# LeapLabTHU/LAUDNet

Hardware: AMD Instinct MI355X
Metric: images/sec, LAUD-ResNet101 @224 bs256 (dynamic-inference hot path) (higher is better)
Workload: dtype bf16x3 (fp32 tensors; each fp32 product = 3 bf16 MFMA products of hi/lo splits, fp32 accumulate)

## Files before the change

include/ldn_hip.h:

```cpp
#ifndef LDN_HIP_H
#define LDN_HIP_H

#include <stddef.h>
#include <stdint.h>

#ifdef __cplusplus
extern "C" {
#endif

#define LDN_OK 0
#define LDN_EINVAL (-1)
#define LDN_EHIP (-2)

const char* ldn_last_error(void);
int ldn_version(void);
int ldn_debug_violations(int* count, int* first_code, int reset);
int ldn_plan_timeouts(int* count, int reset);
const int* ldn_fault_flag(void);
int ldn_device_cus(int* cus);
#define LDN_MATH_DEFAULT (-1)
#define LDN_MATH_FP32 0
#define LDN_MATH_BF16X3 1
int ldn_default_math_mode(void);

// ... 91 lines not shown
                             const float* chan_mask, const int32_t* row_prefix, int B, const int32_t* m_count, int m_cap, int C, float* h,
                             int ldh, void* stream);

size_t ldn_rows_bn_postmask_bwd_workspace_bytes(int m_cap, int C, int B);
int ldn_rows_bn_postmask_bwd(const float* dz, int lddz, const float* u, int ldu, const float* h, int ldh, const float* mean, const float* invstd,
                             const float* gamma, const float* beta, const float* chan_mask, const int32_t* row_prefix, int B, const float* gate,
                             const float* dsq, const int32_t* m_count, int m_cap, int C, float* du, int lddu, float* d_gamma, float* d_beta,
                             float* g_mask, float* work, void* stream);

size_t ldn_rows_ln_bwd_workspace_bytes(int m_cap, int C);
int ldn_rows_ln_bwd(const float* x, int ldx, int rows, const float* stats, const float* gamma, const int32_t* list, const int32_t* count,
                    int m_cap, int C, const float* dy, int lddy, float* dx, int lddx, float* d_gamma, float* d_beta, float* xhat, int ldxh,
                    float* work, void* stream);

int ldn_conv_rows_pool(const float* a, int lda, const int32_t* a_rows, const int32_t* m_count, int m_cap, const void* w,
                       int cin, int cout, const float* scale, const float* shift, int relu, const int32_t* relu_if_neg,
                       const int32_t* out_rows, const float* residual, int ldr, float* out, int ldo, float* pool, int S,
                       int Sx, int Ho, int Wo, int math_mode, void* stream);

int ldn_conv_rows_ps(const float* a, int lda, int a_presplit, const int32_t* a_rows, const int32_t* m_count, int m_cap,
                     const void* w_split, int cin, int cout, const float* scale, const float* shift, int relu,
                     const int32_t* relu_if_neg, const int32_t* out_rows, const float* residual, int ldr, float* out, int ldo,
                     int out_presplit, float* pool, int S, int Sx, int Ho, int Wo, void* stream);
int ldn_conv3x3_rows_ps(const void* a_presplit, int lda, const int32_t* nbr, const int32_t* m_count, int m_cap, const void* w_split,
                        int cin, int cout, const float* scale, const float* shift, int relu, void* out, int ldo, int out_presplit,
                        int rows_hint, void* stream);
int ldn_row_stats(const float* x, int ld, int rows, int C, float eps, float* stats, void* stream);
int ldn_row_stats_list(const float* x, int ld, int rows, int C, float eps, const int32_t* list, const int32_t* count, float* stats,
                       void* stream);

int ldn_channel_masker_splits(int HW);
int ldn_channel_masker(const float* x, int B, int HW, int C, const float* w1, const float* b1, const float* w2,
                       const float* b2, int hidden, int G, int gran, const float* mask_in, float* mask,
                       float* logits, int32_t* ch_idx, int32_t* ch_cnt, float* work, const float* gap_partial,
                       int gap_splits, void* stream);
size_t ldn_channel_masker_workspace_bytes(int B, int HW, int C);

int ldn_forward_stats(const int32_t* cnt, int B, const float* denom, const float* st_in, int st_cols, const double* terms,
                      double static_flops, int n_blocks, float* st_out, float* perc, float* flops, void* stream);

int ldn_conv_image(const float* a, int lda, int B, int Hi, int Wi, int ksize, int stride, int Ho, int Wo,
                   const float* w, int cin, int cout, const int32_t* k_idx, const int32_t* k_cnt, int kgran,
                   const int32_t* n_idx, const int32_t* n_cnt, const float* scale, const float* shift,
                   int shift_classes, const float* post_sub, int relu, const float* residual, int ldr,
                   float* out, int ldo, float* colsum, int out_format, int math_mode, void* stream);

// ... 132 lines not shown
```

laudnet_amd/_lib.py:

```python
from __future__ import annotations

import ctypes as C
import os

import torch

_PKG = os.path.dirname(os.path.abspath(__file__))
LIB_PATH = os.environ.get("LDN_LIB_PATH", os.path.join(_PKG, "libldn_hip.so"))

_P = C.c_void_p
_I = C.c_int

SIGNATURES = {
    "ldn_last_error": ([], C.c_char_p),
    "ldn_version": ([], _I),
    "ldn_debug_violations": ([C.POINTER(_I), C.POINTER(_I), _I], _I),
    "ldn_plan_timeouts": ([C.POINTER(_I), _I], _I),
    "ldn_fault_flag": ([], C.POINTER(_I)),
    "ldn_device_cus": ([C.POINTER(_I)], _I),
    "ldn_default_math_mode": ([], _I),
    "ldn_spatial_masker": ([_P, _I, _I, _I, _I, _P, _P, _I, _I, _P, _P, _P, _P, _P, _P], _I),
    "ldn_spatial_masker_workspace_bytes": ([_I, _I, _I, _I, _I], C.c_size_t),
    "ldn_mask_to_index": ([_P, _I, _I, _I, _I, _I, _I, _P, _P, _P, _P, _P, _P, _P, _P, _P, _P, _P], _I),
    "ldn_mask_to_index_workspace_bytes": ([_I, _I, _I, _I], C.c_size_t),
    "ldn_mask_plan_fits": ([_I, _I, _I, _I, _I], _I),
    "ldn_hint_rows": ([_I], _I),
    "ldn_layer_index": ([_P, _I, _I, _I, _I, _I, _I, _P, _P, _P, _P, _P, _P, _P, _P, _P, _P], _I),
    "ldn_layer_head": ([_P, _I, _I, _I, _P, _P, _I, _P, _P, _P], _I),
    "ldn_mask_plan": ([_P, _P, _I, _P, _P, _P, _P, _I, _I, _I, _I, _I, _I, _I, _P, _P, _P, _P, _P, _P, _P, _P, _P, _P, _P], _I),
    "ldn_conv_rows_pool": ([_P, _I, _P, _P, _I, _P, _I, _I, _P, _P, _I, _P, _P, _P, _I, _P, _I, _P, _I, _I, _I, _I, _I, _P], _I),
    "ldn_conv_rows_ps": ([_P, _I, _I, _P, _P, _I, _P, _I, _I, _P, _P, _I, _P, _P, _P, _I, _P, _I, _I, _P, _I, _I, _I, _I, _P], _I),
    "ldn_conv3x3_rows_ps": ([_P, _I, _P, _P, _I, _P, _I, _I, _P, _P, _I, _P, _I, _I, _I, _P], _I),
    "ldn_gather_rows": ([_P, _I, _P, _P, _I, _I, _P, _I, _P], _I),
    "ldn_scatter_add_relu": ([_P, _I, _P, _P, _I, _I, _P, _I, _P, _I, _P], _I),
    "ldn_conv_rows": ([_P, _I, _P, _I, _P, _I, _P, _I, _I, _P, _P, _I, _P, _P, _P, _I, _P, _I, _I, _P], _I),
    "ldn_conv_rows_split": ([_P, _I, _P, _I, _P, _I, _P, _I, _I, _P, _P, _I, _P, _P, _P, _I, _P, _I, _P, _P, _I, _I, _P, _I, _I, _I,
                             _I, _I, _P, _P, _P], _I),
    "ldn_conv_rows_f32": ([_P, _I, _P, _I, _P, _I, _P, _I, _I, _P, _P, _I, _P, _P, _P, _I, _P, _I, _P, _P, _I, _I, _P, _I, _I, _I,
                             _I, _I, _P, _P, _P], _I),
    "ldn_wgrad_rows_ok": ([_I, _I, _I], _I),
    "ldn_wgrad_rows_workspace_bytes": ([_I, _I, _I, _I], C.c_size_t),
    "ldn_wgrad_rows": ([_P, _I, _P, _I, _I, _P, _I, _P, _I, _I, _I, _P, _P, _I, _P], _I),
    "ldn_wgrad_grouped_rows_ok": ([_I, _I], _I),
    "ldn_wgrad_grouped_rows_workspace_bytes": ([_I, _I, _I], C.c_size_t),
    "ldn_wgrad_grouped_rows": ([_P, _I, _P, _I, _I, _P, _P, _I, _I, _I, _P, _P, _I, _P], _I),
    "ldn_rows_chanmask": ([_P, _I, _P, _I, _P, _P, _I, _I, _P], _I),
    "ldn_rows_act_bwd_workspace_bytes": ([_I, _I, _I], C.c_size_t),
    "ldn_rows_act_bwd": ([_P, _I, _P, _I, _P, _P, _P, _P, _P, _I, _P, _I, _P, _I, _I, _P, _I, _P, _P, _P, _P, _P], _I),
    "ldn_rows_img_dot_workspace_bytes": ([_I, _I, _I], C.c_size_t),
    "ldn_rows_img_dot": ([_P, _I, _P, _I, _P, _I, _P, _I, _I, _P, _P, _P], _I),
    "ldn_rows_postmask_bwd_workspace_bytes": ([_I, _I, _I], C.c_size_t),
    "ldn_rows_postmask_bwd": ([_P, _I, _P, _I, _P, _P, _P, _P, _I, _P, _P, _P, _I, _I, _P, _I, _P, _P, _P, _P, _P], _I),
    "ldn_rows_bn_stats_workspace_bytes": ([_I, _I], C.c_size_t),
    "ldn_rows_bn_stats": ([_P, _I, _P, _P, _I, _P, _I, _I, C.c_float, _P, _P, _P, _P, _P], _I),
# ... 152 lines not shown
```

laudnet_amd/csrc/ldn_dense.hip:

```cpp
#include "ldn_common.h"
#include "ldn_dense_plan.h"
#include <type_traits>

namespace ldn {

struct DenseArgs {
    const float* a; int lda;
    const int32_t* a_rows; const int32_t* m_count; int m_cap;
    const unsigned char* ws;
    int cin, cout;
    const float* scale; const float* shift; int relu;
    const int32_t* relu_if_neg; const int32_t* out_rows;
    const float* residual; int ldr; float* out; int ldo;
    int taps;
    int shift_classes; const int32_t* pix_map;
    int Hi, Wi, Ho, Wo, stride;
    const float* post_sub;
    const float* chmask; int rows_per_img;
    int mtn, ntn;
    const float* ln_stats; const float* ln_c1;
    float* pool; int pool_gy, pool_gx, pool_Sx;
    const float* a_gate; int gate_rows;
};

__device__ __attribute__((aligned(16))) float g_dense_zero[2048] = {0.f};
#ifdef LDN_TRACE
__device__ unsigned long long* g_dense_trace = nullptr;
#define DT(x) x = __builtin_amdgcn_s_memtime();
#else
#define DT(x)
#endif

#ifndef LDN_DENSE_ABLATE
#define LDN_DENSE_ABLATE 0
#endif
__device__ __forceinline__ void dma16_abl(const void* gsrc, unsigned lds_base) {
#if LDN_DENSE_ABLATE & 1
    return;
#endif
#if LDN_DENSE_ABLATE & 2
    gsrc = g_dense_zero;
#endif
    dma16(gsrc, lds_base);
}

// ... 388 lines not shown
        DT(d5)
        a_wait += d1 - d0; a_bar += d2 - d1; a_issue += d3 - d2; a_prep += d4 - d3; a_mfma += d5 - d4;
#endif
    }
#undef LDN_DENSE_STEP
#ifdef LDN_TRACE
    DT(d_loop)
#endif
    wait_vm<0>();
    lds_barrier();
    if (!active) return;

    dense_epilogue<NSUB, T9, FULL, OF>(p, acc, s_arow, s_orow, s_cls, reinterpret_cast<float*>(s_ring + wave * 4096), wave, lane, n0, nsub);
#if defined(LDN_TRACE)
    if (g_dense_trace && lane == 0) {
        unsigned long long dend;
        DT(dend)
        unsigned long long* r = g_dense_trace + ((size_t)blockIdx.x * 8 + wave) * 8;
        r[0] = a_wait; r[1] = a_bar; r[2] = a_issue; r[3] = a_prep; r[4] = a_mfma; r[5] = d_loop - d_start; r[6] = dend - d_loop; r[7] = nchunks;
    }
#endif
}

template <int NSUB, bool T9, bool PS, bool OF, bool FEAT = false, bool RAG = false, bool AG = false>
__global__ __launch_bounds__(512, 2) void k_dense2(const DenseArgs p) {
    static_assert(!RAG || (!T9 && !PS && !OF), "the ragged form is the plain 1x1");
    static_assert(!AG || (!T9 && !PS), "the gated form reads fp32 rows of a 1x1");
    constexpr int NT = NSUB * 32;
    constexpr int KS = NSUB <= 4 ? 64 : 32;
    constexpr int SPS = KS / 32;
    constexpr int WROWB = KS * 4;
    constexpr int UPR = WROWB / 16;
    constexpr int RPI = 1024 / WROWB;
    constexpr int NWI = (NT + 8 * RPI - 1) / (8 * RPI);
    constexpr int WSLOT = NWI * 8 * 1024;
    constexpr int RSLOT = 32 * 128;
    constexpr int D_ROWS = 256, NST = 2 * NSUB;
    extern __shared__ __attribute__((aligned(16))) unsigned char smem[];
    int* const s_arow = reinterpret_cast<int*>(smem);
    int* const s_orow = s_arow + D_ROWS;
    int* const s_cls = s_orow + D_ROWS;
    int* const s_atap = s_cls + D_ROWS;
    unsigned char* const s_w = smem + (T9 ? 12 : 2) * D_ROWS * 4;
    unsigned char* const s_r = s_w + 2 * WSLOT;
    float* const s_gate = reinterpret_cast<float*>(s_r + 8 * 2 * RSLOT);

    const int tid = threadIdx.x, lane = tid & 63;
    const int wave = __builtin_amdgcn_readfirstlane(tid >> 6);
    const int l31 = lane & 31, h = lane >> 5;
    const int xcd = blockIdx.x & 7, slot_i = blockIdx.x >> 3;
    const int nt = slot_i % p.ntn, mt = (slot_i / p.ntn) * 8 + xcd;
    if (mt >= p.mtn) return;
    const int M = p.m_count ? min(p.m_count[0], p.m_cap) : p.m_cap;
    const int m0 = mt * D_ROWS;
    if (m0 >= M) return;
    const int rows = min(D_ROWS, M - m0);
    const int n0 = nt * NT;

    if (tid < D_ROWS) {
        int ar = -1, orw = -1;
        if (tid < rows) {
            ar = (p.a_rows && !T9) ? p.a_rows[m0 + tid] : m0 + tid;
            orw = p.out_rows ? p.out_rows[m0 + tid] : m0 + tid;
            if (p.relu == 1 || (p.relu == 2 && p.relu_if_neg[m0 + tid] < 0)) orw |= D_ROW_RELU;
        }
        int cls = 0;
        if (T9 && tid < rows && p.shift_classes > 1) {
            const int q = p.pix_map[m0 + tid] % (p.Ho * p.Wo);
            const int oy = q / p.Wo, ox = q - oy * p.Wo;
            const int top = oy * p.stride - 1 < 0, bot = oy * p.stride + 1 >= p.Hi;
            const int lef = ox * p.stride - 1 < 0, rig = ox * p.stride + 1 >= p.Wi;
            cls = ((top | (bot << 1)) * 4 + (lef | (rig << 1))) * p.cout;
        }
        LDN_DCHECK(tid >= rows || (ar >= -1 && (orw & (D_ROW_RELU - 1)) >= 0), 501);
        s_arow[tid] = ar;
        s_orow[tid] = orw;
        if (T9) s_cls[tid] = cls;
    }
    if (T9) {
        constexpr int NE = (D_ROWS * 9 + 511) / 512;
        int tv[NE];
#pragma unroll
        for (int u = 0; u < NE; ++u) {
            const int i = tid + 512 * u, r = i / 9;
            tv[u] = (i < D_ROWS * 9 && r < rows) ? p.a_rows[(size_t)(m0 + r) * 9 + (i - r * 9)] : -1;
        }
#pragma unroll
        for (int u = 0; u < NE; ++u)
            if (tid + 512 * u < D_ROWS * 9) s_atap[tid + 512 * u] = tv[u];
    }
    int goff = 0;
    if constexpr (AG) {
        const int gld = round_up(p.cin, 32), q4 = gld >> 2;
        const int slot0 = m0 / p.gate_rows, nsl = (m0 + rows - 1) / p.gate_rows - slot0 + 1;
        for (int i = tid; i < nsl * q4; i += 512) {
            const int sl = i / q4, k = (i - sl * q4) * 4;
            reinterpret_cast<f32x4*>(s_gate)[i] = k < p.cin ? *reinterpret_cast<const f32x4*>(p.a_gate + (size_t)(slot0 + sl) * p.cin + k) : f32x4{0.f, 0.f, 0.f, 0.f};
        }
        goff = ((m0 + min(wave * 32 + (lane & 31), rows - 1)) / p.gate_rows - slot0) * gld + 8 * (lane >> 5);
    }
// ... 7 lines not shown
    const unsigned lds_w = lds_off(s_w), lds_r = lds_off(s_r) + (unsigned)wave * 2u * RSLOT;
    unsigned char* const my_r = s_r + wave * 2 * RSLOT;
    const unsigned char* const zrow = reinterpret_cast<const unsigned char*>(g_dense_zero);

    const unsigned char* wsrc[NWI];
    int wku[NWI];
#pragma unroll
    for (int k = 0; k < NWI; ++k) {
        wku[k] = 0;
        const int rr = 8 * RPI * k + RPI * wave + lane / UPR;
        const int sw = UPR == 16 ? (rr & 15) : ((rr >> 1) & 7);
        wsrc[k] = (rr < NT && (!RAG || n0 + rr < p.cout)) ? p.ws + (long)(n0 + rr) * wrow + (((lane % UPR) ^ sw) << 4) : zrow;
        if (RAG) wku[k] = ((lane % UPR) ^ sw) * 4;
    }
    auto dma_w = [&](int S, int k) {
        const bool pad = NT % (8 * RPI) != 0 && 8 * RPI * k + RPI * wave >= NT;
        const int Sc = min(S, nstep - 1);
        const bool ktail = RAG && Sc * KS + wku[k] >= p.cin;
        dma16_abl(ktail ? zrow : wsrc[k] + (pad || wsrc[k] == zrow ? 0l : (long)Sc * WROWB),
                (unsigned)__builtin_amdgcn_readfirstlane((int)(lds_w + (unsigned)(S & 1) * WSLOT + (unsigned)(8 * RPI * k + RPI * wave) * WROWB)));
    };
    const unsigned char* rsrc[4];
    int tap_r = 0, ck_r = 0;
    auto load_tap = [&](int tap) {
#pragma unroll
        for (int k = 0; k < 4; ++k) {
            const int r = 8 * k + (lane >> 3);
            const int ar = T9 ? s_atap[(wave * 32 + r) * 9 + tap] : s_arow[wave * 32 + r];
            const unsigned char* base = ar >= 0 ? reinterpret_cast<const unsigned char*>(p.a) + (long)ar * p.lda * 4 : zrow;
            rsrc[k] = base + (((lane & 7) ^ ((r >> 1) & 7)) << 4);
        }
    };
    auto dma_r = [&](int s, int k) {
        const unsigned dst = (unsigned)__builtin_amdgcn_readfirstlane((int)(lds_r + (unsigned)(s & 1) * RSLOT + (unsigned)k * 1024u));
        if constexpr (RAG) {
            const int r = 8 * k + (lane >> 3);
            const int ku = ((lane & 7) ^ ((r >> 1) & 7)) * 4;
            dma16_abl(ck_r * 32 + ku < p.cin ? rsrc[k] + ck_r * 128 : zrow, dst);
        } else {
            dma16_abl(rsrc[k] + ck_r * 128, dst);
        }
    };
    auto next_r = [&]() {
        if constexpr (RAG) { ++ck_r; return; }
        if (++ck_r == cpt) {
            ck_r = 0;
            if (T9) {
                tap_r = min(tap_r + 1, 8);
                load_tap(tap_r);
            }
        }
    };

    if (!active) {
        for (int k = 0; k < NWI; ++k) dma_w(0, k);
        for (int S = 0; S < nstep; ++S) {
            wait_vm<0>();
            lds_barrier();
            for (int k = 0; k < NWI; ++k) dma_w(S + 1, k);
        }
        wait_vm<0>();
        return;
    }

    f32x16 acc[NSUB];
#pragma unroll
    for (int j = 0; j < NSUB; ++j)
#pragma unroll
        for (int r = 0; r < 16; ++r) acc[j][r] = 0.f;

    bf16x8 bh[2][2], bl[2][2];
    f32x4 raw[4];
// ... 160 lines not shown
LDN_DEFINE_TU_VIOLATIONS(tu_violations_dense)

static int launch_rows(void (*kernel)(const DenseArgs), const char* name, int r, int nt, unsigned threads, size_t lds, DenseArgs& a, hipStream_t st) {
    a.ntn = ceil_div(a.cout, nt);
    a.mtn = ceil_div(a.m_cap, r);
    LDN_REQUIRE(allow_dynamic_lds(reinterpret_cast<const void*>(kernel), lds), "%s: cannot reserve %zu B of LDS", name, lds);
    hipLaunchKernelGGL(kernel, dim3((unsigned)round_up(a.mtn, 8) * a.ntn), dim3(threads), lds, st, a);
    LDN_CHECK_LAUNCH(name);
    return LDN_OK;
}

template <int NSUB, bool T9, bool FULL, bool F32, int R, bool PS, bool OF>
static int launch_dense_f(DenseArgs& a, hipStream_t st) {
    constexpr int NT = NSUB * 32, D = (NSUB >= 6 || R == 128) ? 2 : 3;
    return launch_rows(&k_dense<NSUB, T9, FULL, F32, R, PS, OF>, "k_dense", R, NT, 2 * R, (size_t)(T9 ? 12 : 2) * R * 4 + (size_t)D * (R + NT) * 128, a, st);
}

template <int NSUB, bool T9, bool PS, bool OF, bool FEAT, bool RAG, bool AG>
static int launch_dense2(DenseArgs& a, hipStream_t st) {
    constexpr int NT = NSUB * 32, KS = NSUB <= 4 ? 64 : 32, WROWB = KS * 4, RPI = 1024 / WROWB, NWI = (NT + 8 * RPI - 1) / (8 * RPI);
    const size_t lds = (size_t)(T9 ? 12 : 2) * 256 * 4 + 2 * (size_t)NWI * 8 * 1024 + 8 * 2 * (size_t)32 * 128 +
                       (AG ? (size_t)dense_gate_bytes(a.gate_rows, a.cin) : 0);
    return launch_rows(&k_dense2<NSUB, T9, PS, OF, FEAT, RAG, AG>, "k_dense2", 256, NT, 512, lds, a, st);
}

static int launch_dense_plan(const DensePlan& plan, DenseArgs& a, hipStream_t st) {
#define LDN_D1(...) if (plan == LDN_DENSE_ROW1(__VA_ARGS__)) return launch_dense_f<__VA_ARGS__>(a, st);
#define LDN_D2(...) if (plan == LDN_DENSE_ROW2(__VA_ARGS__)) return launch_dense2<__VA_ARGS__>(a, st);
    LDN_DENSE_KERNELS(LDN_D1, LDN_D2)
#undef LDN_D1
#undef LDN_D2
    LDN_REQUIRE(false, "ldn_conv_rows: %s is not built (taps %d, cin %d, cout %d, m_cap %d)", dense_plan_name(plan).c_str(), a.taps, a.cin, a.cout, a.m_cap);
}

}

using namespace ldn;

#ifdef LDN_TRACE
extern "C" int ldn_debug_set_dense_trace(void* buf) {
    unsigned long long* q = static_cast<unsigned long long*>(buf);
    return hipMemcpyToSymbol(HIP_SYMBOL(g_dense_trace), &q, sizeof(q)) == hipSuccess ? 0 : -2;
}
#endif

static thread_local long g_rows_hint = -1;
// ... 37 lines not shown
    s.rows_known = dense_rows_known(d.m_cap, d.m_count != nullptr, hint);
    s.f32 = f.f32; s.ps = f.ps; s.of = f.of; s.pool = d.pool != nullptr;
    s.feat = d.post_sub || d.chmask || d.ln_stats || d.relu == 3;
    s.gated = d.a_gate != nullptr; s.gate_bytes = s.gated ? dense_gate_bytes(d.gate_rows, d.cin) : 0;
    return launch_dense_plan(dense_plan(s), d, static_cast<hipStream_t>(stream));
}

extern "C" int ldn_conv_rows_split(const float* a, int lda, const int32_t* a_rows, int taps, const int32_t* m_count, int m_cap,
                                   const void* w_split, int cin, int cout, const float* scale, const float* shift, int relu,
                                   const int32_t* relu_if_neg, const int32_t* out_rows, const float* residual, int ldr,
                                   float* out, int ldo, const float* post_sub, const float* chan_mask, int rows_per_image,
                                   int shift_classes, const int32_t* pix_map, int Hi, int Wi, int Ho, int Wo, int stride,
                                   const float* ln_stats, const float* ln_c1, void* stream) {
    DenseArgs d{};
    d.a = a; d.lda = lda; d.a_rows = a_rows; d.taps = taps; d.m_count = m_count; d.m_cap = m_cap;
    d.ws = static_cast<const unsigned char*>(w_split); d.cin = cin; d.cout = cout;
    d.scale = scale; d.shift = shift; d.relu = relu; d.relu_if_neg = relu_if_neg;
    d.out_rows = out_rows; d.residual = residual; d.ldr = ldr; d.out = out; d.ldo = ldo;
    d.post_sub = post_sub; d.chmask = chan_mask; d.rows_per_img = rows_per_image; d.ln_stats = ln_stats; d.ln_c1 = ln_c1;
    d.shift_classes = shift_classes; d.pix_map = pix_map; d.Hi = Hi; d.Wi = Wi; d.Ho = Ho; d.Wo = Wo; d.stride = stride;
    return conv_rows_dense(d, DenseForm{}, stream);
}

extern "C" int ldn_conv_rows_f32(const float* a, int lda, const int32_t* a_rows, int taps, const int32_t* m_count, int m_cap,
                                 const float* w, int cin, int cout, const float* scale, const float* shift, int relu,
                                 const int32_t* relu_if_neg, const int32_t* out_rows, const float* residual, int ldr,
                                 float* out, int ldo, const float* post_sub, const float* chan_mask, int rows_per_image,
                                 int shift_classes, const int32_t* pix_map, int Hi, int Wi, int Ho, int Wo, int stride,
                                 const float* ln_stats, const float* ln_c1, void* stream) {
    DenseArgs d{};
    d.a = a; d.lda = lda; d.a_rows = a_rows; d.taps = taps; d.m_count = m_count; d.m_cap = m_cap;
    d.ws = reinterpret_cast<const unsigned char*>(w); d.cin = cin; d.cout = cout;
    d.scale = scale; d.shift = shift; d.relu = relu; d.relu_if_neg = relu_if_neg;
    d.out_rows = out_rows; d.residual = residual; d.ldr = ldr; d.out = out; d.ldo = ldo;
    d.post_sub = post_sub; d.chmask = chan_mask; d.rows_per_img = rows_per_image; d.ln_stats = ln_stats; d.ln_c1 = ln_c1;
    d.shift_classes = shift_classes; d.pix_map = pix_map; d.Hi = Hi; d.Wi = Wi; d.Ho = Ho; d.Wo = Wo; d.stride = stride;
    DenseForm f{};
    f.f32 = true;
    return conv_rows_dense(d, f, stream);
}

extern "C" int ldn_conv_rows_pool(const float* a, int lda, const int32_t* a_rows, const int32_t* m_count, int m_cap, const void* w,
                                  int cin, int cout, const float* scale, const float* shift, int relu, const int32_t* relu_if_neg,
                                  const int32_t* out_rows, const float* residual, int ldr, float* out, int ldo, float* pool, int S,
                                  int Sx, int Ho, int Wo, int math_mode, void* stream) {
    LDN_REQUIRE(pool, "ldn_conv_rows_pool: null pool");
// ... 76 lines not shown
```

laudnet_amd/csrc/ldn_dense_plan.h:

```cpp
#pragma once
#include <initializer_list>
#include <stdio.h>
#include <string>

namespace ldn {

struct DenseShape {
    int taps, cin, cout, m_cap;
    long rows_known;
    bool f32, ps, of, pool, feat, gated;
    long gate_bytes;
};

struct DensePlan {
    bool dense2;
    int nsub, rows;
    bool full, feat, rag, t9, f32, ps, of, ag;
};
inline bool operator==(const DensePlan& a, const DensePlan& b) {
    return a.dense2 == b.dense2 && a.nsub == b.nsub && a.rows == b.rows && a.full == b.full && a.feat == b.feat && a.rag == b.rag && a.t9 == b.t9 &&
           a.f32 == b.f32 && a.ps == b.ps && a.of == b.of && a.ag == b.ag;
}
inline std::string dense_plan_name(const DensePlan& p) {
    char s[64];
// ... 11 lines not shown
    D1(2, 0, 0, 1, 256, 0, 0) D1(2, 0, 1, 1, 256, 0, 0) D1(4, 0, 0, 1, 256, 0, 0) D1(4, 0, 1, 1, 256, 0, 0) D1(5, 0, 0, 1, 256, 0, 0)                         \
    D1(5, 0, 1, 1, 256, 0, 0) D1(8, 0, 1, 1, 256, 0, 0) D1(2, 1, 0, 1, 256, 0, 0) D1(2, 1, 1, 1, 256, 0, 0) D1(4, 1, 0, 1, 256, 0, 0) D1(4, 1, 1, 1, 256, 0, 0)\
    D2(2, 0, 0, 0, 0, 0, 0) D2(4, 0, 0, 0, 0, 0, 0) D2(5, 0, 0, 0, 0, 0, 0) D2(6, 0, 0, 0, 0, 0, 0) D2(8, 0, 0, 0, 0, 0, 0)                                   \
    D2(2, 0, 0, 0, 1, 0, 0) D2(4, 0, 0, 0, 1, 0, 0) D2(5, 0, 0, 0, 1, 0, 0) D2(6, 0, 0, 0, 1, 0, 0) D2(8, 0, 0, 0, 1, 0, 0)                                   \
    D2(2, 0, 0, 0, 1, 1, 0) D2(5, 0, 0, 0, 1, 1, 0) D2(2, 1, 0, 0, 0, 0, 0) D2(4, 1, 0, 0, 0, 0, 0)                                                           \
    D2(2, 0, 1, 0, 0, 0, 0) D2(4, 0, 1, 0, 0, 0, 0) D2(8, 0, 1, 0, 0, 0, 0) D2(2, 0, 0, 1, 0, 0, 0) D2(4, 0, 0, 1, 0, 0, 0) D2(8, 0, 0, 1, 0, 0, 0)           \
    D2(2, 0, 0, 0, 1, 1, 1) D2(4, 0, 0, 0, 1, 1, 1) D2(5, 0, 0, 0, 1, 1, 1)
#define LDN_DENSE_ROW1(NSUB, T9, FULL, F32, R, PS, OF) ::ldn::DensePlan{false, NSUB, R, bool(FULL), false, false, bool(T9), bool(F32), bool(PS), bool(OF), false}
#define LDN_DENSE_ROW2(NSUB, T9, PS, OF, FEAT, RAG, AG) ::ldn::DensePlan{true, NSUB, 256, true, bool(FEAT), bool(RAG), bool(T9), false, bool(PS), bool(OF), bool(AG)}

constexpr int kDenseTileRows = 256;
inline long dense_rows_known(int m_cap, bool counted, long hint) { return !counted ? (long)m_cap : (hint >= 0 ? (hint < m_cap ? hint : (long)m_cap) : -1); }
inline long dense_gate_bytes(int gate_rows, int cin) { return (long)(255 / gate_rows + 2) * ((cin + 31) / 32 * 32) * 4; }
constexpr long kChunkCycles = 1700, kChunkCyclesPerSub = 500, kSubtileCycles = 12000, kDenseCus = 256;
constexpr int kShortK = 32, kShortK5 = 144;
constexpr long kWideMinWorkgroups = 384;
constexpr long kGatedWideLds = 30 * 1024;

inline bool dense2_ok(int ns, int taps, int cin, int cout) { return cout % (ns * 32) == 0 && cin % 64 == 0 && cin <= 2048 && (taps == 1 || ns <= 4); }
inline bool dense2_rag_ok(int ns, int cin) { return cin <= 2048 && (ns == 5 || (ns == 2 && cin > 64)); }
inline bool dense_tiles5(int cout) { return cout % 160 == 0 || (cout % 32 != 0 && cout > 128); }
inline bool dense_wide_ok(const DenseShape& s) { return s.cout % 256 == 0 && (long)((s.m_cap + kDenseTileRows - 1) / kDenseTileRows) * (s.cout / 256) >= kWideMinWorkgroups; }

inline double dense_tile_cost(const DenseShape& s, int ns) {
    const long chunks = (long)s.taps * ((s.cin + 31) / 32), wgs = (s.rows_known + kDenseTileRows - 1) / kDenseTileRows * (s.cout / (ns * 32));
    return (double)((wgs + kDenseCus - 1) / kDenseCus) * (double)(chunks * (kChunkCycles + kChunkCyclesPerSub * ns) + kSubtileCycles * ns);
}
inline int dense_cheapest(const DenseShape& s, std::initializer_list<int> widths) {
    int best = 0;
    for (int ns : widths)
        if (s.rows_known > 0 && s.cout % (ns * 32) == 0 && (!best || dense_tile_cost(s, ns) < dense_tile_cost(s, best))) best = ns;
    return best;
}
inline int dense_default_width(const DenseShape& s) { return dense_wide_ok(s) ? 8 : s.cout % 128 == 0 ? 4 : s.cout <= 64 ? 2 : dense_tiles5(s.cout) ? 5 : 4; }

inline DensePlan dense_plan_v1(const DenseShape& s, int ns, int rows = kDenseTileRows) { return {false, ns, rows, s.cout % (ns * 32) == 0, false, false, s.taps == 9, s.f32, s.ps, s.of, s.gated}; }
inline DensePlan dense_plan_v2(const DenseShape& s, int ns, bool feat, bool rag) { return {true, ns, kDenseTileRows, rag || s.cout % (ns * 32) == 0, feat, rag, s.taps == 9, s.f32, s.ps, s.of, s.gated}; }
inline DensePlan dense_plan_whole(const DenseShape& s, int ns) { return dense2_ok(ns, s.taps, s.cin, s.cout) ? dense_plan_v2(s, ns, s.feat && s.taps == 1, false) : dense_plan_v1(s, ns); }

inline DensePlan dense_plan(const DenseShape& s) {
    const bool gate_fits4 = (s.cout % 128 == 0 || (s.cout > 64 && s.cout <= 128)) && s.gate_bytes <= kGatedWideLds;
    if (s.gated) return dense_plan_v2(s, gate_fits4 ? 4 : s.cout <= 64 ? 2 : 5, true, true);
    if (s.taps == 9) {
        const int ns = (s.cout % 128 == 0 ? !s.f32 && dense_cheapest(s, {4, 2}) == 2 : s.cout <= 64) ? 2 : 4;
        return s.f32 ? dense_plan_v1(s, ns) : dense_plan_whole(s, ns);
    }
    if (s.f32) return dense_plan_v1(s, dense_default_width(s));
    if (s.ps || s.of) {
        const int ns = dense_cheapest(s, {8, 4, 2});
        return dense_plan_whole(s, ns ? ns : dense_wide_ok(s) ? 8 : s.cout % 128 == 0 ? 4 : 2);
    }
    if (!s.feat && s.cin <= kShortK && (s.cout <= 64 || s.cout % 128 == 0)) return dense_plan_v1(s, s.cout <= 64 ? 2 : 4, 128);
    if (!s.feat && s.cin <= kShortK5 && dense_tiles5(s.cout)) return dense_plan_v1(s, 5, 128);
    const int best = dense_cheapest(s, {8, 6, 5, 4, 2}), ns = best ? best : dense_default_width(s);
    if (!best && ns == 5 && s.cin <= 2048) return dense_plan_v2(s, 5, true, true);
    if (!dense2_ok(ns, 1, s.cin, s.cout) && dense2_rag_ok(ns, s.cin)) return dense_plan_v2(s, ns, true, true);
    return dense_plan_whole(s, ns);
// ... 4 lines not shown
```

laudnet_amd/laud_resnet.py:

```python
from __future__ import annotations

import itertools
import os

import torch
import torch.nn as nn
import torch.nn.functional as F

from . import ops
from ._lib import LdnError
from ._shared import (channel_constants, dense_channel_convs, dense_index, denoms, flops_constants, identity_residual, rows_hint,
                      sparse_flops, strided_rows)


def _pair(v):
    return tuple(v) if isinstance(v, (tuple, list)) else (v, v)

__all__ = ["uni_resnet50", "uni_resnet101", "ResNet", "Bottleneck", "Masker_spatial", "Masker_channel_MLP",
           "Masker_channel_conv_linear", "ExpandMask"]


def conv3x3(in_planes, out_planes, stride=1, groups=1, dilation=1):
    return nn.Conv2d(in_planes, out_planes, 3, stride=stride, padding=dilation, groups=groups, bias=False,
                     dilation=dilation)
# ... 353 lines not shown

    def _finish_channel(self, out, mask, cnt, gap_out):
        self.last_channel_mask = mask
        self.last_gap = gap_out
        self.last_channel_cnt = cnt
        return ops.from_nhwc(out), mask

    def _run_channel_dense(self, x, p, gap_in=None):
        B, Cin, Hi, Wi = x.shape
        W, gran = self.width, self.channel_dyn_granularity
        Ho, Wo = (Hi - 1) // self.stride + 1, (Wi - 1) // self.stride + 1
        xn = ops.as_nhwc(x)
        mask, _, cnt = self._channel_lists(x, gap_in)
        chm2d = (mask.unsqueeze(2).expand(-1, -1, gran).reshape(B, W) if gran > 1 else mask).contiguous()
        dev = x.device
        if "w2_nk" not in p:
            with torch.no_grad():
                p["w2_nk"] = self.conv2.weight.detach().float().permute(0, 2, 3, 1).reshape(W, 9, W).contiguous().to(dev)
                p["w3_nk"] = p["w3s"].reshape(-1, 1, W)
        ix = dense_index(B, Ho, Wo, self.stride, dev)
        _, h2 = dense_channel_convs(xn.reshape(B * Hi * Wi, Cin), B, (Hi, Wi, Ho, Wo, self.stride), p["w1"], p["w2_nk"], p["s1"], p["t1"],
                                    p["c1"], p["s2"], p["t2_tab"], p["c2"], chm2d, ix)
        cout = p["w3_nk"].shape[0]
        if self.downsample is not None:
            identity = torch.empty(B, Ho, Wo, cout, device=dev, dtype=torch.float32)
            self._shortcut(xn, p, identity)
            out = identity
        else:
            identity = xn
            out = xn if self._inplace else torch.empty_like(xn)
        ops.conv_rows(h2, p["w3_nk"], None, p["t3c"], out.view(B * Ho * Wo, cout), taps=1, m_cap=ix.cap3, relu=1,
                      residual2d=identity.view(B * Ho * Wo, cout))
        return self._finish_channel(out, mask, cnt, None)

    use_fused_head = True
    fused_head_widths = tuple(int(t) for t in os.environ.get("LDN_HEAD_WIDTHS", "64,128,256").split(","))
    use_fused_tail = True

    use_strided_tail = os.environ.get("LDN_TAIL_STRIDE2", "1") != "0"
    use_folded_projection = os.environ.get("LDN_FOLD_PROJ", "1") != "0"

    def _tail_eligible(self, Hi, Wi, Ho, Wo, cout):
        st = self.stride
        return (self.use_fused_tail and self.channel_exec in ("auto", "fused") and ops.fused_kernel_ok()
                and (ops.get_math_mode() != "fp32" or self.conv1.in_channels % 32 == 0)
                and (st == 1 or (st == 2 and self.use_strided_tail)) and (Ho, Wo) == ((Hi - 1) // st + 1, (Wi - 1) // st + 1)
                and self.channel_dyn_granularity % 2 == 0
                and self.width in (64, 128, 256) and Wo <= 256 and cout % 64 == 0
                and ops.bottleneck_tail_splits(Hi, Wi, self.width, st) > 0)

    use_smallmap = os.environ.get("LDN_SMALLMAP", "1") != "0"

    def _smallmap_eligible(self, Cin, Hi, Wi):
        cout = self.conv3.out_channels
        return (self.use_smallmap and self.channel_exec in ("auto", "smallmap") and ops.get_math_mode() == "bf16x3"
                and self.stride == 1 and self.downsample is None and Cin == cout and self.channel_dyn_granularity % 2 == 0
# ... 752 lines not shown
```

laudnet_amd/ops.py:

```python
from __future__ import annotations

import contextlib
import os
import threading
import weakref
from dataclasses import dataclass

import torch

from . import _lib as L


def _f32c(t, what):
    if t is None:
        return None
    if t.dtype != torch.float32 or not t.is_contiguous():
        raise L.LdnError(f"{what}: expected a contiguous float32 tensor, got {t.dtype} strides {t.stride()}")
    return t


def _f32rows(t, what):
    if t is None:
        return None
    if t.dtype != torch.float32 or t.dim() != 2 or t.stride(1) != 1 or t.data_ptr() % 16 != 0:
# ... 397 lines not shown
        return out2d
    if dense_ok:
        hi, wi, ho, wo, stride = geom if geom is not None else (0, 0, 0, 0, 1)
        fn, wptr = ((lib.ldn_conv_rows_split, split_rows_weight(w)) if mode == "bf16x3" else (lib.ldn_conv_rows_f32, _f32c(w, "w")))
        L.check(fn(L.ptr(_f32rows(a2d, "a")), a2d.stride(0), L.ptr(_i32c(a_rows, "a_rows")), taps,
                                        L.ptr(_i32c(m_count, "m_count")), m_cap, L.ptr(wptr), cin, cout,
                                        L.ptr(_f32c(scale, "scale")), L.ptr(_f32c(shift, "shift")), relu,
                                        L.ptr(_i32c(relu_if_neg, "relu_if_neg")), L.ptr(_i32c(out_rows, "out_rows")),
                                        L.ptr(_f32rows(residual2d, "residual")), residual2d.stride(0) if residual2d is not None else 0,
                                        L.ptr(_f32rows(out2d, "out")), out2d.stride(0), L.ptr(_f32c(post_sub, "post_sub")),
                                        L.ptr(_f32c(chan_mask, "chan_mask")), rows_per_image, classes, L.ptr(_i32c(pix_map, "pix_map")),
                                        hi, wi, ho, wo, stride, L.ptr(_f32c(ln_stats, "ln_stats")), L.ptr(_f32c(ln_c1, "ln_c1")),
                                        L.stream_ptr(out2d)), "ldn_conv_rows_split" if mode == "bf16x3" else "ldn_conv_rows_f32")
        return out2d
    L.check(lib.ldn_conv_rows(L.ptr(_f32c(a2d, "a")), a2d.stride(0), L.ptr(_i32c(a_rows, "a_rows")), taps,
                              L.ptr(_i32c(m_count, "m_count")), m_cap, L.ptr(_f32c(w, "w")), cin, cout,
                              L.ptr(_f32c(scale, "scale")), L.ptr(_f32c(shift, "shift")), relu,
                              L.ptr(_i32c(relu_if_neg, "relu_if_neg")), L.ptr(_i32c(out_rows, "out_rows")),
                              L.ptr(_f32rows(residual2d, "residual")), residual2d.stride(0) if residual2d is not None else 0,
                              L.ptr(_f32rows(out2d, "out")), out2d.stride(0), _mm(math), L.stream_ptr(out2d)), "ldn_conv_rows")
    return out2d


def wgrad_rows_ok(cin, cout, taps):
    return bool(L.load().ldn_wgrad_rows_ok(int(cin), int(cout), int(taps)))


def wgrad_rows(dy2d, a2d, *, a_rows=None, taps=1, m_count=None, m_cap=None, a_valid=None, out=None, math=None):
    L.require_device(dy2d, a2d, a_rows, m_count, out)
    lib = L.load()
    cout, cin = dy2d.shape[1], a2d.shape[1]
    if taps not in (1, 9):
        raise L.LdnError(f"wgrad_rows: taps must be 1 or 9, got {taps}")
    if m_cap is None:
        m_cap = dy2d.shape[0] if a_rows is None else a_rows.numel() // taps
    if m_cap > dy2d.shape[0] or (a_rows is not None and a_rows.numel() < m_cap * taps):
        raise L.LdnError(f"wgrad_rows: m_cap {m_cap} exceeds dy2d ({dy2d.shape[0]} rows) or a_rows")
    if a_valid is None:
        a_valid = a2d.shape[0]
    if a_valid > a2d.shape[0] or (a_rows is None and m_cap > a_valid):
        raise L.LdnError(f"wgrad_rows: a_valid {a_valid} / m_cap {m_cap} exceed a2d ({a2d.shape[0]} rows)")
    if out is None:
        out = torch.empty(cout, taps, cin, device=dy2d.device, dtype=torch.float32)
    elif tuple(out.shape) != (cout, taps, cin):
        raise L.LdnError(f"wgrad_rows: out must be [{cout}, {taps}, {cin}], got {tuple(out.shape)}")
    work = _work(lib.ldn_wgrad_rows_workspace_bytes(m_cap, cin, cout, taps), dy2d.device)
# ... 1028 lines not shown
```

Before: 23310.

## Fuse downsample shortcut into conv3 via two-source concatenated-K dense kernel

Adds a two-source variant of the dense 1x1 kernel. It reads the first K-range from the conv2 output rows and the second K-range from strided rows of the block input. For downsampling bottlenecks, the conv3 weight and the BN-scaled shortcut weight are concatenated along K and their shifts summed, so conv3, the shortcut conv and the residual add run as one GEMM launch. This removes the separate identity tensor write and read and one launch. The fused weights are cached on first use, and the path assumes the m_cap row-compaction semantics match (m_cap = B*Ho*Wo).

```diff
diff --git a/include/ldn_hip.h b/include/ldn_hip.h
--- a/include/ldn_hip.h
+++ b/include/ldn_hip.h
@@ -137,6 +137,9 @@
                      const void* w_split, int cin, int cout, const float* scale, const float* shift, int relu,
                      const int32_t* relu_if_neg, const int32_t* out_rows, const float* residual, int ldr, float* out, int ldo,
                      int out_presplit, float* pool, int S, int Sx, int Ho, int Wo, void* stream);
+int ldn_conv_rows_two_width(int cin1, int cin2, int cout, int m_cap);
+int ldn_conv_rows_two(const float* a, int lda, const float* a2, int lda2, const int32_t* a_rows2, int m_cap, const void* w_split,
+                      int cin1, int cin2, int cout, const float* shift, int relu, float* out, int ldo, void* stream);
 int ldn_conv3x3_rows_ps(const void* a_presplit, int lda, const int32_t* nbr, const int32_t* m_count, int m_cap, const void* w_split,
                         int cin, int cout, const float* scale, const float* shift, int relu, void* out, int ldo, int out_presplit,
                         int rows_hint, void* stream);
diff --git a/laudnet_amd/_lib.py b/laudnet_amd/_lib.py
--- a/laudnet_amd/_lib.py
+++ b/laudnet_amd/_lib.py
@@ -30,6 +30,8 @@
     "ldn_mask_plan": ([_P, _P, _I, _P, _P, _P, _P, _I, _I, _I, _I, _I, _I, _I, _P, _P, _P, _P, _P, _P, _P, _P, _P, _P, _P], _I),
     "ldn_conv_rows_pool": ([_P, _I, _P, _P, _I, _P, _I, _I, _P, _P, _I, _P, _P, _P, _I, _P, _I, _P, _I, _I, _I, _I, _I, _P], _I),
     "ldn_conv_rows_ps": ([_P, _I, _I, _P, _P, _I, _P, _I, _I, _P, _P, _I, _P, _P, _P, _I, _P, _I, _I, _P, _I, _I, _I, _I, _P], _I),
+    "ldn_conv_rows_two_width": ([_I, _I, _I, _I], _I),
+    "ldn_conv_rows_two": ([_P, _I, _P, _I, _P, _I, _P, _I, _I, _I, _P, _I, _P, _I, _P], _I),
     "ldn_conv3x3_rows_ps": ([_P, _I, _P, _P, _I, _P, _I, _I, _P, _P, _I, _P, _I, _I, _I, _P], _I),
     "ldn_gather_rows": ([_P, _I, _P, _P, _I, _I, _P, _I, _P], _I),
     "ldn_scatter_add_relu": ([_P, _I, _P, _P, _I, _I, _P, _I, _P, _I, _P], _I),
diff --git a/laudnet_amd/csrc/ldn_dense.hip b/laudnet_amd/csrc/ldn_dense.hip
--- a/laudnet_amd/csrc/ldn_dense.hip
+++ b/laudnet_amd/csrc/ldn_dense.hip
@@ -21,6 +21,9 @@
     const float* ln_stats; const float* ln_c1;
     float* pool; int pool_gy, pool_gx, pool_Sx;
     const float* a_gate; int gate_rows;
+};
+struct DenseArgsTwo : DenseArgs {
+    const float* a2; int lda2; const int32_t* a_rows2; int cin1;
 };
 
 __device__ __attribute__((aligned(16))) float g_dense_zero[2048] = {0.f};
@@ -455,9 +458,10 @@
 #endif
 }
 
-template <int NSUB, bool T9, bool PS, bool OF, bool FEAT = false, bool RAG = false, bool AG = false>
-__global__ __launch_bounds__(512, 2) void k_dense2(const DenseArgs p) {
+template <int NSUB, bool T9, bool PS, bool OF, bool FEAT = false, bool RAG = false, bool AG = false, bool TWO = false>
+__global__ __launch_bounds__(512, 2) void k_dense2(const std::conditional_t<TWO, DenseArgsTwo, DenseArgs> p) {
     static_assert(!RAG || (!T9 && !PS && !OF), "the ragged form is the plain 1x1");
+    static_assert(!TWO || (!T9 && !PS && !OF && !RAG && !AG), "the two-source form is the plain 1x1 over fp32 rows");
     static_assert(!AG || (!T9 && !PS), "the gated form reads fp32 rows of a 1x1");
     constexpr int NT = NSUB * 32;
     constexpr int KS = NSUB <= 4 ? 64 : 32;
@@ -473,8 +477,9 @@
     int* const s_arow = reinterpret_cast<int*>(smem);
     int* const s_orow = s_arow + D_ROWS;
     int* const s_cls = s_orow + D_ROWS;
+    int* const s_arow2 = s_cls;
     int* const s_atap = s_cls + D_ROWS;
-    unsigned char* const s_w = smem + (T9 ? 12 : 2) * D_ROWS * 4;
+    unsigned char* const s_w = smem + (T9 ? 12 : TWO ? 3 : 2) * D_ROWS * 4;
     unsigned char* const s_r = s_w + 2 * WSLOT;
     float* const s_gate = reinterpret_cast<float*>(s_r + 8 * 2 * RSLOT);
 
@@ -509,6 +514,7 @@
         s_arow[tid] = ar;
         s_orow[tid] = orw;
         if (T9) s_cls[tid] = cls;
+        if constexpr (TWO) s_arow2[tid] = tid < rows ? (p.a_rows2 ? p.a_rows2[m0 + tid] : m0 + tid) : -1;
     }
     if (T9) {
         constexpr int NE = (D_ROWS * 9 + 511) / 512;
@@ -562,12 +568,17 @@
     };
     const unsigned char* rsrc[4];
     int tap_r = 0, ck_r = 0;
+    int cpt_r = cpt;
+    if constexpr (TWO) cpt_r = p.cin1 >> 5;
     auto load_tap = [&](int tap) {
 #pragma unroll
         for (int k = 0; k < 4; ++k) {
             const int r = 8 * k + (lane >> 3);
-            const int ar = T9 ? s_atap[(wave * 32 + r) * 9 + tap] : s_arow[wave * 32 + r];
+            const int ar = T9 ? s_atap[(wave * 32 + r) * 9 + tap] : (TWO && tap) ? s_arow2[wave * 32 + r] : s_arow[wave * 32 + r];
             const unsigned char* base = ar >= 0 ? reinterpret_cast<const unsigned char*>(p.a) + (long)ar * p.lda * 4 : zrow;
+            if constexpr (TWO) {
+                if (tap && ar >= 0) base = reinterpret_cast<const unsigned char*>(p.a2) + (long)ar * p.lda2 * 4;
+            }
             rsrc[k] = base + (((lane & 7) ^ ((r >> 1) & 7)) << 4);
         }
     };
@@ -583,11 +594,16 @@
     };
     auto next_r = [&]() {
         if constexpr (RAG) { ++ck_r; return; }
-        if (++ck_r == cpt) {
+        if (++ck_r == (TWO ? cpt_r : cpt)) {
             ck_r = 0;
             if (T9) {
                 tap_r = min(tap_r + 1, 8);
                 load_tap(tap_r);
+            }
+            if constexpr (TWO) if (tap_r == 0) {
+                tap_r = 1;
+                cpt_r = cpt - (p.cin1 >> 5);
+                load_tap(1);
             }
         }
     };
@@ -794,6 +810,19 @@
     const size_t lds = (size_t)(T9 ? 12 : 2) * 256 * 4 + 2 * (size_t)NWI * 8 * 1024 + 8 * 2 * (size_t)32 * 128 +
                        (AG ? (size_t)dense_gate_bytes(a.gate_rows, a.cin) : 0);
     return launch_rows(&k_dense2<NSUB, T9, PS, OF, FEAT, RAG, AG>, "k_dense2", 256, NT, 512, lds, a, st);
+}
+
+template <int NSUB>
+static int launch_dense2_two(DenseArgsTwo& a, hipStream_t st) {
+    constexpr int NT = NSUB * 32, KS = NSUB <= 4 ? 64 : 32, WROWB = KS * 4, RPI = 1024 / WROWB, NWI = (NT + 8 * RPI - 1) / (8 * RPI);
+    const size_t lds = (size_t)3 * 256 * 4 + 2 * (size_t)NWI * 8 * 1024 + 8 * 2 * (size_t)32 * 128;
+    auto kernel = &k_dense2<NSUB, false, false, false, false, false, false, true>;
+    a.ntn = ceil_div(a.cout, NT);
+    a.mtn = ceil_div(a.m_cap, 256);
+    LDN_REQUIRE(allow_dynamic_lds(reinterpret_cast<const void*>(kernel), lds), "k_dense2<two>: cannot reserve %zu B of LDS", lds);
+    hipLaunchKernelGGL(kernel, dim3((unsigned)round_up(a.mtn, 8) * a.ntn), dim3(512), lds, st, a);
+    LDN_CHECK_LAUNCH("k_dense2<two>");
+    return LDN_OK;
 }
 
 static int launch_dense_plan(const DensePlan& plan, DenseArgs& a, hipStream_t st) {
@@ -877,6 +906,26 @@
     return conv_rows_dense(d, DenseForm{}, stream);
 }
 
+extern "C" int ldn_conv_rows_two_width(int cin1, int cin2, int cout, int m_cap) { return dense_two_width(cin1, cin2, cout, m_cap); }
+extern "C" int ldn_conv_rows_two(const float* a, int lda, const float* a2, int lda2, const int32_t* a_rows2, int m_cap, const void* w_split,
+                                 int cin1, int cin2, int cout, const float* shift, int relu, float* out, int ldo, void* stream) {
+    LDN_REQUIRE(a && a2 && w_split && shift && out, "ldn_conv_rows_two: null pointer");
+    LDN_REQUIRE(m_cap >= 0 && (relu == 0 || relu == 1), "ldn_conv_rows_two: bad m_cap / relu (0 none, 1 ReLU)");
+    const int ns = dense_two_width(cin1, cin2, cout, m_cap > 0 ? m_cap : 1);
+    LDN_REQUIRE(ns != 0, "ldn_conv_rows_two: cin1 %d, cin2 %d, cout %d is not a shape of the two-source form (cin1, cin2 multiples of 64 and <= 2048, cout of 128)", cin1, cin2, cout);
+    LDN_REQUIRE(lda % 4 == 0 && lda >= cin1 && lda2 % 4 == 0 && lda2 >= cin2 && ldo % 4 == 0 && ldo >= cout, "ldn_conv_rows_two: strides must be multiples of 4 and cover the row");
+    LDN_REQUIRE((uintptr_t)a % 16 == 0 && (uintptr_t)a2 % 16 == 0 && (uintptr_t)w_split % 16 == 0 && (uintptr_t)out % 16 == 0 && (uintptr_t)shift % 16 == 0,
+                "ldn_conv_rows_two: pointers must be 16-byte aligned");
+    if (m_cap == 0) return LDN_OK;
+    DenseArgsTwo d{};
+    d.a = a; d.lda = lda; d.taps = 1; d.m_cap = m_cap; d.ws = static_cast<const unsigned char*>(w_split); d.cin = cin1 + cin2; d.cout = cout;
+    d.shift = shift; d.relu = relu; d.out = out; d.ldo = ldo; d.shift_classes = 1;
+    d.Ho = d.Wo = d.rows_per_img = d.gate_rows = 1;
+    d.a2 = a2; d.lda2 = lda2; d.a_rows2 = a_rows2; d.cin1 = cin1;
+    hipStream_t st = static_cast<hipStream_t>(stream);
+    return ns == 8 ? launch_dense2_two<8>(d, st) : launch_dense2_two<4>(d, st);
+}
+
 extern "C" int ldn_conv_rows_f32(const float* a, int lda, const int32_t* a_rows, int taps, const int32_t* m_count, int m_cap,
                                  const float* w, int cin, int cout, const float* scale, const float* shift, int relu,
                                  const int32_t* relu_if_neg, const int32_t* out_rows, const float* residual, int ldr,
diff --git a/laudnet_amd/csrc/ldn_dense_plan.h b/laudnet_amd/csrc/ldn_dense_plan.h
--- a/laudnet_amd/csrc/ldn_dense_plan.h
+++ b/laudnet_amd/csrc/ldn_dense_plan.h
@@ -57,6 +57,10 @@
 inline bool dense_tiles5(int cout) { return cout % 160 == 0 || (cout % 32 != 0 && cout > 128); }
 inline bool dense_wide_ok(const DenseShape& s) { return s.cout % 256 == 0 && (long)((s.m_cap + kDenseTileRows - 1) / kDenseTileRows) * (s.cout / 256) >= kWideMinWorkgroups; }
 
+inline bool dense2_two_ok(int ns, int cin1, int cin2, int cout) {
+    return (ns == 4 || ns == 8) && cin1 > 0 && cin2 > 0 && cin1 % 64 == 0 && cin2 % 64 == 0 && cin1 <= 2048 && cin2 <= 2048 && cout > 0 && cout % (ns * 32) == 0;
+}
+
 inline double dense_tile_cost(const DenseShape& s, int ns) {
     const long chunks = (long)s.taps * ((s.cin + 31) / 32), wgs = (s.rows_known + kDenseTileRows - 1) / kDenseTileRows * (s.cout / (ns * 32));
     return (double)((wgs + kDenseCus - 1) / kDenseCus) * (double)(chunks * (kChunkCycles + kChunkCyclesPerSub * ns) + kSubtileCycles * ns);
@@ -68,6 +72,13 @@
     return best;
 }
 inline int dense_default_width(const DenseShape& s) { return dense_wide_ok(s) ? 8 : s.cout % 128 == 0 ? 4 : s.cout <= 64 ? 2 : dense_tiles5(s.cout) ? 5 : 4; }
+
+inline int dense_two_width(int cin1, int cin2, int cout, int m_cap) {
+    if (m_cap <= 0 || !dense2_two_ok(4, cin1, cin2, cout)) return 0;
+    DenseShape s{};
+    s.taps = 1; s.cin = cin1 + cin2; s.cout = cout; s.m_cap = m_cap; s.rows_known = m_cap;
+    return dense2_two_ok(8, cin1, cin2, cout) && dense_tile_cost(s, 8) < dense_tile_cost(s, 4) ? 8 : 4;
+}
 
 inline DensePlan dense_plan_v1(const DenseShape& s, int ns, int rows = kDenseTileRows) { return {false, ns, rows, s.cout % (ns * 32) == 0, false, false, s.taps == 9, s.f32, s.ps, s.of, s.gated}; }
 inline DensePlan dense_plan_v2(const DenseShape& s, int ns, bool feat, bool rag) { return {true, ns, kDenseTileRows, rag || s.cout % (ns * 32) == 0, feat, rag, s.taps == 9, s.f32, s.ps, s.of, s.gated}; }
diff --git a/laudnet_amd/laud_resnet.py b/laudnet_amd/laud_resnet.py
--- a/laudnet_amd/laud_resnet.py
+++ b/laudnet_amd/laud_resnet.py
@@ -399,6 +399,16 @@
         _, h2 = dense_channel_convs(xn.reshape(B * Hi * Wi, Cin), B, (Hi, Wi, Ho, Wo, self.stride), p["w1"], p["w2_nk"], p["s1"], p["t1"],
                                     p["c1"], p["s2"], p["t2_tab"], p["c2"], chm2d, ix)
         cout = p["w3_nk"].shape[0]
+        if (self.downsample is not None and self.use_s4_fold and ops.get_math_mode() == "bf16x3" and ops.dense_kernel_ok()
+                and ops.conv_rows_two_width(W, Cin, cout, B * Ho * Wo)):
+            if "w3d" not in p:
+                with torch.no_grad():
+                    p["w3d"] = torch.cat((p["w3s"], p["wd"].reshape(cout, Cin) * p["sd"].view(-1, 1)), dim=1).contiguous()
+                    p["t3cd"] = (p["t3c"] + p["td"]).contiguous()
+            out = torch.empty(B, Ho, Wo, cout, device=dev, dtype=torch.float32)
+            ops.conv_rows_two(h2[:B * Ho * Wo], xn.reshape(B * Hi * Wi, Cin), p["w3d"], p["t3cd"], out.view(B * Ho * Wo, cout),
+                              b_rows=strided_rows(B, Hi, Wi, Ho, Wo, p["ds_stride"], dev), relu=1)
+            return self._finish_channel(out, mask, cnt, None)
         if self.downsample is not None:
             identity = torch.empty(B, Ho, Wo, cout, device=dev, dtype=torch.float32)
             self._shortcut(xn, p, identity)
@@ -409,6 +419,8 @@
         ops.conv_rows(h2, p["w3_nk"], None, p["t3c"], out.view(B * Ho * Wo, cout), taps=1, m_cap=ix.cap3, relu=1,
                       residual2d=identity.view(B * Ho * Wo, cout))
         return self._finish_channel(out, mask, cnt, None)
+
+    use_s4_fold = os.environ.get("LDN_S4_FOLD", "1") != "0"
 
     use_fused_head = True
     fused_head_widths = tuple(int(t) for t in os.environ.get("LDN_HEAD_WIDTHS", "64,128,256").split(","))
diff --git a/laudnet_amd/ops.py b/laudnet_amd/ops.py
--- a/laudnet_amd/ops.py
+++ b/laudnet_amd/ops.py
@@ -443,6 +443,23 @@
     return out2d
 
 
+def conv_rows_two_width(cin1, cin2, cout, rows):
+    return L.load().ldn_conv_rows_two_width(int(cin1), int(cin2), int(cout), int(rows))
+
+
+def conv_rows_two(a2d, b2d, w, shift, out2d, *, b_rows=None, relu=1):
+    L.require_device(a2d, b2d, w, out2d, b_rows)
+    cout, cin = w.shape
+    cin1 = a2d.shape[1]
+    m_cap = out2d.shape[0]
+    if a2d.shape[0] < m_cap or (b_rows is not None and b_rows.numel() < m_cap) or (b_rows is None and b2d.shape[0] < m_cap) or out2d.shape[1] != cout:
+        raise L.LdnError("conv_rows_two: a2d / b_rows must cover the rows of out2d [rows, cout]")
+    L.check(L.load().ldn_conv_rows_two(L.ptr(_f32rows(a2d, "a")), a2d.stride(0), L.ptr(_f32rows(b2d, "b")), b2d.stride(0), L.ptr(_i32c(b_rows, "b_rows")),
+                                       m_cap, L.ptr(split_rows_weight(w)), cin1, cin - cin1, cout, L.ptr(_f32c(shift, "shift")), relu,
+                                       L.ptr(_f32rows(out2d, "out")), out2d.stride(0), L.stream_ptr(out2d)), "ldn_conv_rows_two")
+    return out2d
+
+
 def wgrad_rows_ok(cin, cout, taps):
     return bool(L.load().ldn_wgrad_rows_ok(int(cin), int(cout), int(taps)))
 
```

New measurement: 23330, median of 3. No clear change (+0.1%).
